# nkwangyh/CubemapSLAM

Measured on AMD Instinct MI355X. Metric: frames/sec (extract+match+localBA) on Lafida cam0, higher is better.
Workload: dtype u8 (extract/match), f64 (BA)

## Files before the change

cubemapslam_amd/csrc/cms_api_ba.hip:

```cpp
#include <algorithm>
#include <cfloat>
#include <chrono>
#include <condition_variable>
#include <deque>
#include <functional>
#include <atomic>
#include <cmath>
#include <mutex>
#include <numeric>
#include <string>
#include <thread>
#include <pthread.h>
#include <unordered_map>
#include "cms_ba_pool.h"

struct BaKnobs {
  bool deterministic, det_points, host_lm, single_host_lm, schur_chunks, schur_points, all_lists, want_all_lists;
  bool no_fused, solve1, trial_points, fixed_ranges, no_permute, create_timing, compose_timing, runs, runs_as_edges, separate_reduce, separate_reduce2, separate_first_pass, rm_valu;
  int solve_reduce_max, leftover_lookahead;
  bool global_sum;
  int lookahead, compose_segments, dup, run_min_chunks, rm_weight, se_waves_cap, em_cost_a, em_cost_b, te_chunks, run_min_pct; bool unified;
  char stream_priority;
  bool run_wg; int rw_waves_cu0, rw_waves_cu1;
};
static const BaKnobs& ba_knobs() {
  static const BaKnobs k = [] {
    BaKnobs q;
    auto on = [](const char* n) { return getenv(n) != nullptr; };
    auto num = [](const char* n, int dflt) { const char* v = getenv(n); return v ? atoi(v) : dflt; };
    q.deterministic = on("CMS_BA_DETERMINISTIC"); q.host_lm = on("CMS_BA_HOST_LM"); q.single_host_lm = on("CMS_BA_SINGLE_HOST_LM");
    q.schur_chunks = on("CMS_BA_SCHUR_CHUNKS"); q.schur_points = on("CMS_BA_SCHUR_POINTS"); q.all_lists = on("CMS_BA_ALL_LISTS");
    q.det_points = on("CMS_BA_DET_POINTS");
    q.want_all_lists = (q.deterministic && q.det_points) || q.host_lm || q.single_host_lm || q.schur_chunks || q.schur_points || q.all_lists;
    q.no_fused = on("CMS_BA_NO_FUSED_LIN"); q.solve1 = on("CMS_BA_SOLVE1"); q.trial_points = on("CMS_BA_TRIAL_POINTS");
    q.fixed_ranges = on("CMS_BA_FIXED_RANGES"); q.no_permute = on("CMS_BA_NO_PERMUTE");
    q.create_timing = on("CMS_BA_CREATE_TIMING"); q.compose_timing = on("CMS_BA_COMPOSE_TIMING");
    q.runs = !on("CMS_BA_NO_RUNS");
    q.runs_as_edges = on("CMS_BA_RUNS_AS_EDGES");
    q.rm_valu = on("CMS_BA_RM_VALU");
    q.separate_first_pass = on("CMS_BA_SEPARATE_FIRST_PASS");
    q.separate_reduce2 = on("CMS_BA_SEPARATE_REDUCE2");
    q.separate_reduce = on("CMS_BA_SEPARATE_REDUCE");
    { const char* v = getenv("CMS_BA_SOLVE_REDUCE_MAX"); q.solve_reduce_max = v ? atoi(v) : 24; }
    q.global_sum = !on("CMS_BA_NO_GLOBAL_SUM");
    q.leftover_lookahead = num("CMS_BA_LEFTOVER_LOOKAHEAD", 0);
    q.lookahead = num("CMS_BA_LOOKAHEAD", 24); q.compose_segments = num("CMS_BA_COMPOSE_SEGMENTS", 0); q.dup = num("CMS_BA_DUP", 0);
    q.run_min_chunks = std::max(1, num("CMS_BA_RUN_MIN_CHUNKS", q.rm_valu ? 2 : 1));
    q.run_min_pct = std::max(10, std::min(100, num("CMS_BA_RUN_MIN_PCT", 100)));
    q.rm_weight = std::max(10, std::min(400, num("CMS_BA_RM_WEIGHT", 58)));
    q.unified = !on("CMS_BA_SPLIT_WORKGROUPS");
    q.em_cost_a = num("CMS_BA_EM_COST_A", 40); q.em_cost_b = num("CMS_BA_EM_COST_B", 30);
    q.te_chunks = std::max(1, std::min(16, num("CMS_BA_TE_CHUNKS", 2)));
    q.se_waves_cap = num("CMS_BA_SE_WAVES", 0);
    q.run_wg = on("CMS_BA_RUN_WG");
    q.rw_waves_cu0 = std::max(1, std::min(32, num("CMS_BA_RW_WAVES0", 12))); q.rw_waves_cu1 = std::max(1, std::min(32, num("CMS_BA_RW_WAVES1", 8)));
    const char* pr = getenv("CMS_BA_STREAM_PRIORITY");
    q.stream_priority = pr ? pr[0] : 0;
    return q;
  }();
  return k;
}

struct BaExpand;
struct BaDevPlan;
struct BaCreateOpts {
  hipStream_t setup_stream = nullptr;
  bool inputs_pinned = false;
  bool force_host_plan = false;
  BaDevPlan* dev_plan = nullptr;
  BaExpand* defer_expand = nullptr;
};
struct BaCreated { bool expand_deferred = false; };
struct cms_ba {
  int device = 0;
  hipStream_t stream = nullptr; bool own_stream = true, pooled_stream = false;
  int K = 0, P = 0, E = 0, np = 0, nblk_e = 0, nblk_p = 0;
  std::vector<int> perm;
  std::vector<int> pinv;
  std::vector<int> se_chunk_pt0;
  BaDev d;
  uint8_t* d_fixed = nullptr; int* d_pose_slot = nullptr; int* d_e_pose = nullptr; int* d_e_point = nullptr;
  double* d_e_obs = nullptr; double* d_e_inv = nullptr; int8_t* d_e_face = nullptr; int* d_pt_off = nullptr;
  double* d_raw_obs = nullptr; double* d_raw_inv = nullptr; double* d_raw_pts = nullptr; int* d_perm = nullptr; int* d_pinv = nullptr;
  int* d_pose_off = nullptr; int* d_pose_edges = nullptr; uint8_t* d_level = nullptr; double* d_err = nullptr; double* d_ow = nullptr;
  double* d_poses[2] = {nullptr, nullptr}; double* d_pts[2] = {nullptr, nullptr};
  double* d_poses0 = nullptr; double* d_pts0 = nullptr;
  double* d_Hpp = nullptr; double* d_bp = nullptr; double* d_Hll = nullptr; double* d_bl = nullptr; double* d_Hpl = nullptr;
  double* d_Dinv = nullptr; double* d_Hs = nullptr; double* d_bs = nullptr; double* d_x = nullptr; double* d_Dg = nullptr;
// ... 16 lines not shown
  int cur = 0;
  double* h_pin = nullptr; size_t h_pin_bytes = 0;
  void* grp_items_dev = nullptr; void* grp_items_host = nullptr; double* grp_scal_dev = nullptr; double* grp_scal_host = nullptr;
  void* grp_lm_dev = nullptr; void* grp_lm_host = nullptr;
  int grp_cap = 0;
  int prof_kernel = 0; std::vector<hipEvent_t> prof_ev; double prof_ms = 0; long prof_launches = 0;
  bool fast_plan = false;
  int* d_raw_pose = nullptr; int* d_raw_point = nullptr; int8_t* d_raw_face = nullptr; int* d_prank = nullptr; int* d_cpo = nullptr; int* d_cedge = nullptr;
  uint8_t* d_pcopy = nullptr; uint8_t* d_lo_copy = nullptr; uint64_t* d_run_sig = nullptr; int* d_iperm = nullptr;
  bool dev_plan = false;
  int* d_plan_counts = nullptr; int* h_plan_counts = nullptr; size_t h_plan_counts_bytes = 0;
  long long* d_plan_clk = nullptr;
  bool se_only = false;
  bool deterministic = false;
  int det_ranges = 0;
  bool det_points = false;
  hipEvent_t ev_setup = nullptr;
  bool setup_wait_pending = false;
  hipStream_t grp_stream = nullptr;
  bool async_pending = false;
  bool gsum_clean = false;
  BaSe grp_se = {};
  std::vector<BaBlock> slabs; size_t slab_off = 0;
  size_t grp_pin_bytes[3] = {0, 0, 0};
};

#define BA_LDS_CEILING (160 * 1024 - 512)
static int ba_lds_attrs_once(int device) {
  static std::mutex mu;
  static bool done[64] = {false};
  std::lock_guard<std::mutex> lk(mu);
  if (device < 0 || device >= 64 || done[device]) return CMS_OK;
  const void* fns[] = {(const void*)k_ba_schur_points, (const void*)kb_ba_schur_points, (const void*)kb_ba_schur_edges, (const void*)kb_ba_lin_schur_edges,
                       (const void*)kb_ba_lin_schur_runs, (const void*)kb_ba_lin_schur_runs_det, (const void*)kb_ba_lin_schur_edges_det, (const void*)kb_ba_lin_schur_runs_valu, (const void*)kb_ba_lin_schur_run_wg0, (const void*)kb_ba_lin_schur_run_wg1, (const void*)kb_ba_trial_solve3r, (const void*)kb_ba_trial_solve3rp, (const void*)k_ba_trial_solve,
                       (const void*)kb_ba_trial_solve, (const void*)kb_ba_trial_solve3, (const void*)k_ba_solve_r192};
  for (const void* f : fns) {
    hipError_t e = hipFuncSetAttribute(f, hipFuncAttributeMaxDynamicSharedMemorySize, BA_LDS_CEILING);
    if (e != hipSuccess) return cms_fail(CMS_ERR_HIP, "hipFuncSetAttribute(MaxDynamicSharedMemorySize)", e);
  }
  done[device] = true;
  return CMS_OK;
}

struct BaPools {
  static size_t slab_cap() { const char* v = getenv("CMS_BA_POOL_MB"); return v ? (size_t)std::max(0, atoi(v)) << 20 : (size_t)16 << 30; }
  BaIdleList<hipStream_t> streams{256}, setup_streams{0};
  BaIdleList<hipEvent_t> events{1024};
  BaBlockCache dev{slab_cap(), 0};
  BaBlockCache pin{(size_t)2 << 30, 512}, stage{(size_t)2 << 30, 512};
};
static BaPools& ba_pools() { static BaPools* p = new BaPools; return *p; }
static hipStream_t ba_stream_take(int device) { return ba_pools().streams.take(device); }
static hipError_t ba_wait_stream(hipStream_t s) {
  static const bool relaxed = getenv("CMS_BA_RELAXED_WAIT") != nullptr;
  if (!relaxed) return hipStreamSynchronize(s);
  for (int i = 0; i < 64; ++i) {
    const hipError_t q = hipStreamQuery(s);
    if (q != hipErrorNotReady) return q == hipSuccess ? hipStreamSynchronize(s) : q;
  }
  for (;;) {
    std::this_thread::sleep_for(std::chrono::microseconds(40));
    const hipError_t q = hipStreamQuery(s);
    if (q != hipErrorNotReady) return q == hipSuccess ? hipStreamSynchronize(s) : q;
  }
}
static void ba_stream_give(int device, hipStream_t s) {
  const hipError_t q = hipStreamQuery(s);
  if ((q != hipSuccess && q != hipErrorNotReady) || !ba_pools().streams.give(device, s)) hipStreamDestroy(s);
// ... 1568 lines not shown
```

cubemapslam_amd/csrc/cms_api_ba_lm.hip:

```cpp

struct BaLm {
  int iterations = 0, robust = 0;
  double delta = 0;
  int it = 0, qmax = 0, nBad = 0, done = 0, next = 0;
  double lambda = -1, ni = 2, currentChi = 0, iniChi = 0, rho = 0;
  double chi_ini = 0, chi_fin = 0, lam_fin = 0;
};

static bool ba_stopped(const volatile uint8_t* stop) { return stop && *stop; }

static int ba_enqueue_iter_start(cms_ba* b, const BaLm& st) {
  hipStream_t s = b->stream;
  const int cur = b->cur;
  ba_errors(b, cur, st.robust, st.delta, 0);
  hipLaunchKernelGGL(k_ba_lin_points, dim3(b->nblk_p), dim3(128), 0, s, b->d, (const double*)b->d_poses[cur],
                     (const double*)b->d_pts[cur], st.robust, st.delta, b->d_Hll, b->d_bl, b->d_Hpl);
  hipLaunchKernelGGL(k_ba_lin_poses, dim3(b->K, BA_POSE_CHUNKS), dim3(256), 0, s, b->d, (const double*)b->d_poses[cur],
                     (const double*)b->d_pts[cur], st.robust, st.delta, b->d_pose_partial);
  if (b->np > 0)
    hipLaunchKernelGGL(k_ba_pose_finish, dim3(b->np), dim3(64), 0, s, b->np, (const double*)b->d_pose_partial, b->d_Hpp, b->d_bp);
  if (st.it == 0) {
    HIPCHK(hipMemsetAsync(b->d_scal + 3, 0, sizeof(double), s));
    hipLaunchKernelGGL(k_ba_maxdiag, dim3(64), dim3(256), 0, s, b->np, b->P, (const double*)b->d_Hpp, (const double*)b->d_Hll, b->d_scal + 3);
  }
// ... 338 lines not shown
  BaDyn dyn{};
  memset(&dyn, 0, sizeof(dyn));
  dyn.robust = st[0].robust; dyn.delta = st[0].delta; dyn.chi2_th = 5.991; dyn.set_level = 0; dyn.dev_lm = 1; dyn.fold_finish = 1;
  bool first_round = false;
  for (int w = 0; w < n; ++w) first_round = first_round || st[w].it == 0;
  const BaGroupMode gm = ba_group_mode(bas, n);
  const bool use_se = gm.use_se, use_te = gm.use_te;
  bool iter_phase = true;
  const bool use_s3 = gm.use_s3;
  int s3_threads = 64; size_t lds3 = 0;
  for (int w = 0; w < n; ++w) { s3_threads = std::max(s3_threads, ba_s3_threads(bas[w]->np)); lds3 = std::max(lds3, bas[w]->blk3_lds); }
  {
    static const int solve_kb = [] { const char* v = getenv("CMS_BA_SOLVE_LDS_KB"); return v ? atoi(v) : 0; }();
    if (solve_kb > 0) lds3 = std::max(lds3, std::min((size_t)solve_kb * 1024, (size_t)BA_LDS_CEILING));
  }
  int max_seR = 0, max_np2 = 0, max_Rt = 0; size_t se_lds = 0, te_lds = 0, rm_lds = 0;
  const int se_waves = gm.se_waves;
  bool any_runs = false, any_rw0 = false, any_rw1 = false;
  for (int w = 0; w < n; ++w) {
    const BaSe& gs = bas[w]->grp_se;
    if (gm.run_wg) { any_rw0 = any_rw0 || gs.n_rmA > 0; any_rw1 = any_rw1 || gs.n_rm > gs.n_rmA; }
    max_seR = std::max(max_seR, gs.R_rm + gs.R); max_np2 = std::max(max_np2, gs.npairs2); se_lds = std::max(se_lds, bas[w]->se_lds_fixed);
    any_runs = any_runs || gs.R_rm > 0;
    if (gs.R_rm > 0) rm_lds = std::max(rm_lds, bas[w]->rm_lds);
    max_Rt = std::max(max_Rt, gs.Rt); te_lds = std::max(te_lds, ((size_t)24 * bas[w]->K + 6 * (size_t)std::max(bas[w]->np, 1)) * sizeof(double));
  }
  se_lds += (size_t)se_waves * ((size_t)64 * 18 * sizeof(double) + 64 * sizeof(int));
  se_lds = std::max(se_lds, rm_lds);
  const int se_threads = 64 * se_waves;
  const size_t rw_lds = ba_rw_lds(std::max(max_K, 1));
  const int rw_units0 = std::max(8, std::min(BA_RW_CUTS, ba_device_cus(bas[0]->device) * ba_knobs().rw_waves_cu0 / std::max(n, 1)));
  const int rw_units1 = std::max(8, std::min(BA_RW_CUTS, ba_device_cus(bas[0]->device) * ba_knobs().rw_waves_cu1 / std::max(n, 1)));
  const bool fused = gm.fused;
  const bool solve_reduces = fused && (gm.gsum || (!ba_knobs().separate_reduce && max_seR <= ba_knobs().solve_reduce_max));
  dyn.fused_lin = fused ? 1 : 0;
  {
    static const bool no_presum = getenv("CMS_BA_NO_SOLVE_PRESUM") != nullptr;
    const size_t need = lds3 + (size_t)max_np2 * 42 * sizeof(double);
    if (use_s3 && solve_reduces && !gm.gsum && !no_presum && need <= BA_LDS_CEILING) { dyn.solve_presum = 1; lds3 = need; }
  }
  const bool first_pass = fused && use_te && first_round && !ba_knobs().separate_first_pass;
  dyn.fold_reduce = (use_te && !ba_knobs().separate_reduce2 && ba_knobs().dup == 0) ? 1 : 0;
  int k = 0;
  const int pk = g->prof_kernel;
  const int dup = ba_knobs().dup;
  auto bracket = [&](int id, int which) {
    if (pk != id) return;
    const size_t i = 2 * (size_t)k + which;
    while (g->prof_ev.size() <= i) { hipEvent_t e = nullptr; if (hipEventCreate(&e) != hipSuccess) return; g->prof_ev.push_back(e); }
    hipEventRecord(g->prof_ev[i], s);
  };
  auto enqueue_round = [&]() {
      if (first_round && first_pass) {
        bracket(1, 0);
        hipLaunchKernelGGL(kb_ba_first_pass, dim3(max_Rt, 1, n), dim3(BA_TE_THREADS), te_lds, s, ditems, dyn, (int)BA_PHASE_ITER);
        bracket(1, 1);
        iter_phase = false;
      } else if (first_round) {
        hipLaunchKernelGGL(kb_ba_errors, dim3(max_e, 1, n), dim3(256), 0, s, ditems, dyn, (int)BA_PHASE_ITER);
        hipLaunchKernelGGL(kb_ba_reduce, dim3(1, 1, n), dim3(256), 0, s, ditems, dyn, (int)BA_PHASE_ITER);
      }
      first_round = false;
      if (iter_phase) {
        const int npb = (max_P + 255) / 256;
        bracket(1, 0);
        hipLaunchKernelGGL(kb_ba_lin, dim3(npb + max_K * BA_POSE_CHUNKS, 1, n), dim3(256), 0, s, ditems, dyn, (int)BA_PHASE_ITER, npb);
// ... 15 lines not shown
          if (any_rw1) hipLaunchKernelGGL(kb_ba_lin_schur_run_wg1, dim3(rw_units1, 1, n), dim3(64), rw_lds, s, ditems, dyn, (int)BA_PHASE_TRIAL, rw_units1);
          if (any_rw0) hipLaunchKernelGGL(kb_ba_lin_schur_run_wg0, dim3(rw_units0, 1, n), dim3(64), rw_lds, s, ditems, dyn, (int)BA_PHASE_TRIAL, rw_units0);
          if (max_seR > 0) hipLaunchKernelGGL(kb_ba_lin_schur_edges, dim3(max_seR, 1, n), dim3(se_threads), se_lds, s, ditems, dyn, (int)BA_PHASE_TRIAL);
        } else if (fused && gm.det) {
          if (any_runs) hipLaunchKernelGGL(kb_ba_lin_schur_runs_det, dim3(max_seR, 1, n), dim3(se_threads), se_lds, s, ditems, dyn, (int)BA_PHASE_TRIAL);
          else hipLaunchKernelGGL(kb_ba_lin_schur_edges_det, dim3(max_seR, 1, n), dim3(se_threads), se_lds, s, ditems, dyn, (int)BA_PHASE_TRIAL);
        } else if (fused && any_runs) {
          hipLaunchKernelGGL(kb_ba_lin_schur_runs, dim3(max_seR, 1, n), dim3(se_threads), se_lds, s, ditems, dyn, (int)BA_PHASE_TRIAL);
          if (dup == 3) hipLaunchKernelGGL(kb_ba_lin_schur_runs, dim3(max_seR, 1, n), dim3(se_threads), se_lds, s, ditems, dyn, (int)BA_PHASE_TRIAL);
        } else if (fused) {
          hipLaunchKernelGGL(kb_ba_lin_schur_edges, dim3(max_seR, 1, n), dim3(se_threads), se_lds, s, ditems, dyn, (int)BA_PHASE_TRIAL);
          if (dup == 3) hipLaunchKernelGGL(kb_ba_lin_schur_edges, dim3(max_seR, 1, n), dim3(se_threads), se_lds, s, ditems, dyn, (int)BA_PHASE_TRIAL);
        } else {
          hipLaunchKernelGGL(kb_ba_schur_edges, dim3(max_seR, 1, n), dim3(se_threads), se_lds, s, ditems, dyn, (int)BA_PHASE_TRIAL);
          if (dup == 3) hipLaunchKernelGGL(kb_ba_schur_edges, dim3(max_seR, 1, n), dim3(se_threads), se_lds, s, ditems, dyn, (int)BA_PHASE_TRIAL);
        }
        bracket(3, 1);
        bracket(4, 0);
        if (!solve_reduces) hipLaunchKernelGGL(kb_ba_schur_edges_reduce, dim3(max_np2, 1, n), dim3(256), 0, s, ditems, dyn, (int)BA_PHASE_TRIAL);
        bracket(4, 1);
      } else if (all_sp) {
        bracket(3, 0);
        hipLaunchKernelGGL(kb_ba_schur_points, dim3(max_R, 1, n), dim3(max_spt), sp_lds, s, ditems, dyn, (int)BA_PHASE_TRIAL);
        if (dup == 3) hipLaunchKernelGGL(kb_ba_schur_points, dim3(max_R, 1, n), dim3(max_spt), sp_lds, s, ditems, dyn, (int)BA_PHASE_TRIAL);
        bracket(3, 1);
        bracket(4, 0);
        hipLaunchKernelGGL(kb_ba_schur_reduce, dim3(max_pairs, 1, n), dim3(256), 0, s, ditems, dyn, (int)BA_PHASE_TRIAL);
        if (dup == 4) hipLaunchKernelGGL(kb_ba_schur_reduce, dim3(max_pairs, 1, n), dim3(256), 0, s, ditems, dyn, (int)BA_PHASE_TRIAL);
        bracket(4, 1);
      } else if (max_chunks > 0) {
        hipLaunchKernelGGL(kb_ba_schur_chunks, dim3(max_chunks, 1, n), dim3(256), 0, s, ditems, dyn, (int)BA_PHASE_TRIAL);
      }
      bracket(5, 0);
      if (use_s3 && solve_reduces && dyn.solve_presum) {
        hipLaunchKernelGGL(kb_ba_trial_solve3rp, dim3(1, 1, n), dim3(s3_threads), lds3, s, ditems, dyn, (int)BA_PHASE_TRIAL);
      } else if (use_s3 && solve_reduces) {
        hipLaunchKernelGGL(kb_ba_trial_solve3r, dim3(1, 1, n), dim3(s3_threads), lds3, s, ditems, dyn, (int)BA_PHASE_TRIAL);
        if (dup == 5) hipLaunchKernelGGL(kb_ba_trial_solve3r, dim3(1, 1, n), dim3(s3_threads), lds3, s, ditems, dyn, (int)BA_PHASE_TRIAL);
      } else if (use_s3) {
        hipLaunchKernelGGL(kb_ba_trial_solve3, dim3(1, 1, n), dim3(s3_threads), lds3, s, ditems, dyn, (int)BA_PHASE_TRIAL);
        if (dup == 5) hipLaunchKernelGGL(kb_ba_trial_solve3, dim3(1, 1, n), dim3(s3_threads), lds3, s, ditems, dyn, (int)BA_PHASE_TRIAL);
      } else {
        hipLaunchKernelGGL(kb_ba_trial_solve, dim3(1, 1, n), dim3(384), lds, s, ditems, dyn, (int)BA_PHASE_TRIAL);
        if (dup == 5) hipLaunchKernelGGL(kb_ba_trial_solve, dim3(1, 1, n), dim3(384), lds, s, ditems, dyn, (int)BA_PHASE_TRIAL);
      }
      bracket(5, 1);
      bracket(6, 0);
      if (use_te) {
        hipLaunchKernelGGL(kb_ba_trial_edges, dim3(max_Rt, 1, n), dim3(BA_TE_THREADS), te_lds, s, ditems, dyn, (int)BA_PHASE_TRIAL);
        if (dup == 6) hipLaunchKernelGGL(kb_ba_trial_edges, dim3(max_Rt, 1, n), dim3(BA_TE_THREADS), te_lds, s, ditems, dyn, (int)BA_PHASE_TRIAL);
      } else {
        hipLaunchKernelGGL(kb_ba_trial_points, dim3(max_p, 1, n), dim3(128), 0, s, ditems, dyn, (int)BA_PHASE_TRIAL);
        if (dup == 6) hipLaunchKernelGGL(kb_ba_trial_points, dim3(max_p, 1, n), dim3(128), 0, s, ditems, dyn, (int)BA_PHASE_TRIAL);
      }
      bracket(6, 1);
      bracket(7, 0);
      if (!dyn.fold_reduce) hipLaunchKernelGGL(kb_ba_reduce2, dim3(1, 1, n), dim3(256), 0, s, ditems, dyn, (int)BA_PHASE_TRIAL);
      bracket(7, 1);
      ++k;
  };
  const volatile BaLmDev* vh = reinterpret_cast<const volatile BaLmDev*>(hlm);
  hipError_t werr = hipSuccess;
  for (long spins = 0;;) {
    bool any = false;
    for (int w = 0; w < n; ++w) any = any || vh[w].next != 2;
    if (!any || (k > 0 && ba_stopped(stop))) break;
    if (k - vh[0].rounds < (stop ? 1 : 2)) { enqueue_round(); spins = 0; continue; }
    if (spins < 256) std::this_thread::yield();
    else std::this_thread::sleep_for(std::chrono::microseconds(20));
    if ((++spins & 0xFFF) == 0 && hipStreamQuery(s) != hipErrorNotReady) {
      werr = hipStreamSynchronize(s);
      if (werr != hipSuccess || k - vh[0].rounds >= 2) { if (werr == hipSuccess) werr = hipErrorUnknown; break; }
    }
  }
// ... 168 lines not shown
```

cubemapslam_amd/csrc/cms_ba_fused.hip:

```cpp
#include <hip/hip_runtime.h>
#include <stdint.h>

__device__ __forceinline__ void ba_factor_diag(double* a, int J, double* Ld, double* ybuf, double* idg, int* bad) {
  double idl[6];
#pragma unroll
  for (int c = 0; c < 6; ++c) {
    const double dc = a[7 * c];
    if (!(isfinite(dc)) || dc == 0.0) *bad = 1;
    double x = __builtin_amdgcn_rcp(dc);
    x = __builtin_fma(__builtin_fma(-dc, x, 1.0), x, x);
    x = __builtin_fma(__builtin_fma(-dc, x, 1.0), x, x);
    idl[c] = x;
    double lc[6];
#pragma unroll
    for (int r = c + 1; r < 6; ++r) lc[r] = a[6 * r + c] * x;
#pragma unroll
    for (int r = c + 1; r < 6; ++r) {
#pragma unroll
      for (int q = c + 1; q <= r; ++q) a[6 * r + q] = __builtin_fma(-lc[r], a[6 * q + c], a[6 * r + q]);
    }
#pragma unroll
    for (int r = c + 1; r < 6; ++r) a[6 * r + c] = lc[r];
  }
  double z[6];
#pragma unroll
  for (int r = 0; r < 6; ++r) z[r] = ybuf[6 * J + r];
#pragma unroll
  for (int r = 0; r < 6; ++r) {
#pragma unroll
    for (int c = 0; c < r; ++c) z[r] = __builtin_fma(-a[6 * r + c], z[c], z[r]);
  }
#pragma unroll
  for (int r = 1; r < 6; ++r)
#pragma unroll
    for (int c = 0; c < r; ++c) Ld[6 * r + c] = a[6 * r + c];
#pragma unroll
  for (int r = 0; r < 6; ++r) { ybuf[6 * J + r] = z[r]; idg[6 * J + r] = idl[r]; }
}

__device__ __forceinline__ void ba_trial_pose_update(BaDevG d, const double* ybuf, const double* __restrict__ bp, double lambda, const double* __restrict__ poses,
                                                     double* __restrict__ poses_new, double* __restrict__ scal, bool isbad) {
  const int tid = threadIdx.x;
  double sc = 0;
  for (int k = tid; k < d.K; k += blockDim.x) {
    const double* T = poses + 7 * k;
    double* Tn = poses_new + 7 * k;
    const int s = d.pose_slot[k];
    if (s < 0) { for (int i = 0; i < 7; ++i) Tn[i] = T[i]; continue; }
    const double* u = ybuf + 6 * s;
    for (int i = 0; i < 6; ++i) sc += u[i] * (lambda * u[i] + bp[6 * s + i]);
    const double om[3] = {u[0], u[1], u[2]}, up[3] = {u[3], u[4], u[5]};
    const double theta = sqrt(om[0] * om[0] + om[1] * om[1] + om[2] * om[2]);
    const double Om[9] = {0, -om[2], om[1], om[2], 0, -om[0], -om[1], om[0], 0};
    double Om2[9];
    for (int i = 0; i < 3; ++i)
      for (int j = 0; j < 3; ++j) Om2[3 * i + j] = Om[3 * i] * Om[j] + Om[3 * i + 1] * Om[3 + j] + Om[3 * i + 2] * Om[6 + j];
    double R[9], V[9];
    if (theta < 0.00001) {
      for (int i = 0; i < 9; ++i) { R[i] = ((i & 3) == 0 ? 1.0 : 0.0) + Om[i] + Om2[i]; V[i] = R[i]; }
    } else {
      double sn, cs;
      sincos(theta, &sn, &cs);
      const double sa = sn / theta, sb = (1 - cs) / (theta * theta), scc = (theta - sn) / (theta * theta * theta);
      for (int i = 0; i < 9; ++i) {
        const double Id = ((i & 3) == 0 ? 1.0 : 0.0);
        R[i] = Id + sa * Om[i] + sb * Om2[i];
        V[i] = Id + sb * Om[i] + scc * Om2[i];
      }
    }
    double Eq[4], Et[3], RE[9];
// ... 177 lines not shown
      }
      for (int o = tid; o < 6 * J; o += 64) {
        const int Kq = o / 6, c = o - 6 * Kq;
        const int mq = nb - Kq - 1, iq = J - Kq - 1;
        const double* Lq = Lp + 36 * (size_t)(Kq * nb - Kq * (Kq + 1) / 2);
        double v = ybuf[o];
#pragma unroll
        for (int r = 0; r < 6; ++r) { const int q = 6 * r + c; v -= Lq[((q >> 1) * mq + iq) * 2 + (q & 1)] * xj[r]; }
        ybuf[o] = v;
      }
      __builtin_amdgcn_wave_barrier();
    }
  }
  __syncthreads();
  if (isbad) for (int i = tid; i < n; i += blockDim.x) ybuf[i] = 0.0;
  __syncthreads();
  BA_CLK(3);
  for (int i = tid; i < n; i += blockDim.x) xp_out[i] = ybuf[i];
  ba_trial_pose_update(d, ybuf, bp, lambda, poses, poses_new, scal, isbad);
  BA_CLK(4);
#undef BA_CLK
}

#define BA_S3_STRIDE 38
#define BA_S3_BPW 21
#define BA_S3_NY 3
static inline int ba_s3_threads(int np) { return (np * (np + 1) / 2 + BA_S3_BPW - 1) / BA_S3_BPW * 64; }
#ifdef BA_S3_CLK
__device__ long long ba_s3_clk[16];
#define BA_S3_STAMP(i) do { if (s3_on) { const long long now_ = (long long)__builtin_readcyclecounter(); s3_acc[i] += now_ - s3_last; s3_last = now_; } } while (0)
#else
#define BA_S3_STAMP(i) do { } while (0)
#endif
__device__ __forceinline__ void ba_trial_solve3_body(BaDevG d, const double* __restrict__ Hpp, const double* __restrict__ bp, double lambda,
                 const int* __restrict__ pair_of_block, const int* __restrict__ pair_chunk_off,
                 const double* __restrict__ chunk_sum, const double* __restrict__ poses, double* __restrict__ poses_new,
                 double* __restrict__ xp_out, double* __restrict__ scal, bool lumped = false, double* partial = nullptr,
                 double* bp_partial = nullptr, int n_slices = 0, int NP2 = 0, bool consume = false, bool presum = false) {
  extern __shared__ __align__(16) double sm[];
  const int nb = d.np, n = 6 * nb, nblk = nb * (nb + 1) / 2;
  double* Lp = sm;
  double* Ldg = Lp + (size_t)BA_S3_STRIDE * (nb * (nb - 1) / 2);
  double* Wbuf = Ldg + 36 * (size_t)nb;
  double* dstage = Wbuf + 2 * (size_t)BA_S3_STRIDE * nb;
  double* ybuf = dstage + 36;
  double* idg = ybuf + n;
  double* bps = idg + n;
  double* ssum = bps + n;
  const bool presummed = partial && presum && !consume && n_slices > 1;
  if (presummed) {
    const int tot = NP2 * 42;
    for (int i = threadIdx.x; i < tot; i += blockDim.x) {
      double v = 0.0;
#pragma unroll 8
      for (int r = 0; r < n_slices; ++r) v += partial[(size_t)r * tot + i];
      ssum[i] = v;
    }
    __syncthreads();
  }
#ifdef BA_S3_CLK
  const bool s3_on = threadIdx.x == 0 && blockIdx.z == 0;
  long long s3_acc[10] = {0, 0, 0, 0, 0, 0, 0, 0, 0, 0};
  long long s3_last = (long long)__builtin_readcyclecounter();
#endif
  if (partial) {
    for (int i = threadIdx.x; i < n; i += blockDim.x) {
// ... 44 lines not shown
        if (I == K && consume) {
#pragma unroll
          for (int q = 0; q < 6; ++q) {
            a[q] -= cs[6 * min(q, r0) + max(q, r0)];
            a[6 + q] -= cs[6 * min(q, r0 + 1) + max(q, r0 + 1)];
          }
        } else {
#pragma unroll
          for (int q = 0; q < 6; ++q) { const double2 v = *reinterpret_cast<const double2*>(cs + 6 * q + r0); a[q] -= v.x; a[6 + q] -= v.y; }
        }
        if (I == K) { const double2 v = *reinterpret_cast<const double2*>(cs + 36 + r0); yb[0] += v.x; yb[1] += v.y; }
        if (consume) {
#pragma unroll
          for (int q = 0; q < 6; ++q) *reinterpret_cast<double2*>(cs + 6 * q + r0) = make_double2(0.0, 0.0);
          if (I == K) *reinterpret_cast<double2*>(cs + 36 + r0) = make_double2(0.0, 0.0);
        }
      }
    } else if (pr >= 0) {
      for (int c = pair_chunk_off[pr]; c < pair_chunk_off[pr + 1]; ++c) {
        const double* cs = chunk_sum + (size_t)c * 42;
#pragma unroll
        for (int q = 0; q < 6; ++q) { a[q] -= cs[6 * q + r0]; a[6 + q] -= cs[6 * q + r0 + 1]; }
        if (I == K) { yb[0] += cs[36 + r0]; yb[1] += cs[36 + r0 + 1]; }
      }
    }
    if (I == K) {
      ybuf[6 * I + r0] = (lumped ? 0.0 : bp[6 * I + r0]) - yb[0];
      ybuf[6 * I + r0 + 1] = (lumped ? 0.0 : bp[6 * I + r0 + 1]) - yb[1];
    }
  }
#define BA_S3_WAVE_SYNC() do { __builtin_amdgcn_fence(__ATOMIC_RELEASE, "wavefront"); __builtin_amdgcn_wave_barrier(); \
                               __builtin_amdgcn_fence(__ATOMIC_ACQUIRE, "wavefront"); } while (0)
  if (wave == 0) {
    if (have && I == 0 && K == 0) {
#pragma unroll
      for (int q = 0; q < 12; ++q) dstage[6 * r0 + q] = a[q];
    }
    BA_S3_WAVE_SYNC();
    if (tid == 0) {
      double f[36];
#pragma unroll
      for (int q = 0; q < 36; ++q) f[q] = dstage[q];
      ba_factor_diag(f, 0, Ldg, ybuf, idg, &bad);
    }
  }
  __syncthreads();
  BA_S3_STAMP(0);
  for (int J = 0; J < nb && !bad; ++J) {
    double* Wp = Wbuf + (size_t)(J & 1) * BA_S3_STRIDE * nb;
    double* Lpan = Lp + (size_t)BA_S3_STRIDE * (J * nb - J * (J + 1) / 2);
    if (have && K == J && I > J) {
      const double* Ld = Ldg + 36 * (size_t)J;
      double ld[15], idj[6], zj[6];
#pragma unroll
      for (int c = 1; c < 6; ++c)
#pragma unroll
        for (int q = 0; q < c; ++q) ld[c * (c - 1) / 2 + q] = Ld[6 * c + q];
#pragma unroll
      for (int c = 0; c < 6; ++c) { idj[c] = idg[6 * J + c]; zj[c] = ybuf[6 * J + c]; }
      double yi[2] = {ybuf[6 * I + r0], ybuf[6 * I + r0 + 1]};
      double w[12], lo[12];
#pragma unroll
      for (int r = 0; r < 2; ++r)
#pragma unroll
        for (int c = 0; c < 6; ++c) {
          double v = a[6 * r + c];
#pragma unroll
          for (int q = 0; q < c; ++q) v = __builtin_fma(-w[6 * r + q], ld[c * (c - 1) / 2 + q], v);
          w[6 * r + c] = v;
        }
#pragma unroll
      for (int r = 0; r < 2; ++r)
#pragma unroll
        for (int c = 0; c < 6; ++c) {
          const double l = w[6 * r + c] * idj[c];
          lo[6 * r + c] = l;
          yi[r] = __builtin_fma(-l, zj[c], yi[r]);
        }
      const int i = I - J - 1;
      double2* W2 = reinterpret_cast<double2*>(Wp + (size_t)i * BA_S3_STRIDE + 6 * r0);
      double2* L2 = reinterpret_cast<double2*>(Lpan + (size_t)i * BA_S3_STRIDE + 6 * r0);
#pragma unroll
      for (int q = 0; q < 6; ++q) { W2[q] = make_double2(w[2 * q], w[2 * q + 1]); L2[q] = make_double2(lo[2 * q], lo[2 * q + 1]); }
      ybuf[6 * I + r0] = yi[0]; ybuf[6 * I + r0 + 1] = yi[1];
    }
    __syncthreads();
    BA_S3_STAMP(2);
    const bool next_diag = have && I == J + 1 && K == J + 1;
    const int blkd = (J + 1) * nb - (J + 1) * J / 2, wd = blkd / BA_S3_BPW;
    const bool crit = J + 1 < nb && wave == wd;
    if (crit) __builtin_amdgcn_s_setprio(3);
    if (have && K > J) {
      const int iw = I - J - 1, ik = K - J - 1;
      double wv[12], lk[36];
      const double2* W2 = reinterpret_cast<const double2*>(Wp + (size_t)iw * BA_S3_STRIDE + 6 * r0);
      const double2* L2 = reinterpret_cast<const double2*>(Lpan + (size_t)ik * BA_S3_STRIDE);
#pragma unroll
      for (int q = 0; q < 6; ++q) { const double2 x = W2[q]; wv[2 * q] = x.x; wv[2 * q + 1] = x.y; }
#pragma unroll
      for (int q = 0; q < 18; ++q) { const double2 y = L2[q]; lk[2 * q] = y.x; lk[2 * q + 1] = y.y; }
#pragma unroll
      for (int r = 0; r < 2; ++r)
#pragma unroll
        for (int q = 0; q < 6; ++q) {
          double v = a[6 * r + q];
#pragma unroll
          for (int c = 0; c < 6; ++c) v = __builtin_fma(-wv[6 * r + c], lk[6 * q + c], v);
          a[6 * r + q] = v;
        }
      if (next_diag) {
#pragma unroll
        for (int q = 0; q < 12; ++q) dstage[6 * r0 + q] = a[q];
      }
    }
    if (crit) {
      BA_S3_WAVE_SYNC();
      if (lane == 3 * (blkd - BA_S3_BPW * wd)) {
        double f[36];
#pragma unroll
        for (int q = 0; q < 36; ++q) f[q] = dstage[q];
        ba_factor_diag(f, J + 1, Ldg + 36 * (size_t)(J + 1), ybuf, idg, &bad);
      }
      __builtin_amdgcn_s_setprio(0);
    }
    __syncthreads();
    BA_S3_STAMP(3);
  }
  const bool isbad = bad != 0;
  if (!isbad && wave == 0) {
    const int ln = min(lane, 59);
    double y[BA_S3_NY];
    const double* Lo[BA_S3_NY];
#pragma unroll
    for (int g = 0; g < BA_S3_NY; ++g) {
      const int o = 60 * g + ln;
      y[g] = o < n ? ybuf[o] * idg[o] : 0.0;
      const int Kq = o / 6, c = o - 6 * Kq;
      Lo[g] = Lp + (ptrdiff_t)BA_S3_STRIDE * (Kq * nb - Kq * (Kq + 1) / 2 - Kq - 1) + c;
    }
    const double* Lsafe = Lp - BA_S3_STRIDE;
    double nld[15];
    auto fetch = [&](int J) {
      const double* Ld = Ldg + 36 * (size_t)J;
#pragma unroll
      for (int q = 1; q < 6; ++q)
#pragma unroll
        for (int r = 0; r < q; ++r) nld[q * (q - 1) / 2 + r] = Ld[6 * q + r];
    };
// ... 140 lines not shown
```

cubemapslam_amd/csrc/cms_ba_wrappers.hip:

```cpp
#include <hip/hip_runtime.h>
#include <stdint.h>

#define BA_MAX_GROUP 64
struct BaLmDev {
  double lambda, ni, currentChi, iniChi, rho, chi_ini, chi_fin, lam_fin;
  int it, iterations, qmax, nBad, done, next, cur, rounds;
  int n_out[2], pad[2];
};
struct BaItem {
  BaDev d;
  double* poses[2]; double* pts[2];
  double* Hll; double* bl; double* Hpl; double* Hpp; double* bp; double* pose_partial; double* Dinv; double* db;
  double* chunk_sum; double* x; double* partial; double* scal;
  double* hscal;
  const int2* chunk_range; const int2* tup; const int* pair_of_block; const int* pair_chunk_off;
  uint8_t* flags;
  int nblk_e, nblk_p, nchunks, block_free;
  BaSp sp;
  BaSe se;
  BaLmDev* lm; BaLmDev* hlm;
};
template <class T> struct BaGP {
  BA_AS1 T* p;
  __device__ __forceinline__ BaGP() {}
// ... 241 lines not shown
  ba_schur_edges_body<true, true>(blockIdx.x, it.d, it.se, it.Hll, it.bl, ba_lambda, it.poses[cur], it.pts[cur], dyn.robust, dyn.delta);
}
extern "C" __global__ void __launch_bounds__(BA_SE_THREADS) kb_ba_lin_schur_runs_valu(const BaItem* __restrict__ items, BaDyn dyn, int phase) {
  BA_ITEM(phase, it.se.R_rm + it.se.R)
  if ((int)blockIdx.x < it.se.R_rm) ba_schur_runs_body(blockIdx.x, it.d, it.se, it.Hll, it.bl, ba_lambda, it.poses[cur], it.pts[cur], dyn.robust, dyn.delta);
  else ba_schur_edges_body<true>((int)blockIdx.x - it.se.R_rm, it.d, it.se, it.Hll, it.bl, ba_lambda, it.poses[cur], it.pts[cur], dyn.robust, dyn.delta);
}
extern "C" __global__ void __launch_bounds__(256) kb_ba_schur_edges_reduce(const BaItem* __restrict__ items, BaDyn dyn, int phase) {
  BA_ITEM(phase, it.se.nchunks > 0 ? it.se.npairs2 : 0)
  BaSpG v;
  v.R = it.se.R_rm + it.se.R; v.npairs = it.se.npairs2; v.partial = it.se.partial;
  ba_schur_reduce_body(blockIdx.x, v, it.chunk_sum);
  if (dyn.fused_lin && (int)blockIdx.x < it.d.np) {
    __shared__ double bps[6 * BA_SE_RANGES];
    const int R = min(it.se.R_rm + it.se.R, BA_SE_RANGES);
    for (int t = threadIdx.x; t < 6 * R; t += blockDim.x) bps[t] = it.se.bp_partial[((size_t)(t / 6) * it.d.np + blockIdx.x) * 6 + (t % 6)];
    __syncthreads();
    if (threadIdx.x < 6) {
      double sum = 0.0;
      for (int r = 0; r < R; ++r) sum += bps[6 * r + threadIdx.x];
      it.bp[6 * blockIdx.x + threadIdx.x] = sum;
    }
  }
}
extern "C" __global__ void __launch_bounds__(256) kb_ba_schur_reduce(const BaItem* __restrict__ items, BaDyn dyn, int phase) {
  BA_ITEM(phase, it.sp.R > 0 ? it.sp.npairs : 0)
  ba_schur_reduce_body(blockIdx.x, it.sp, it.chunk_sum);
}
extern "C" __global__ void __launch_bounds__(384) kb_ba_trial_solve(const BaItem* __restrict__ items, BaDyn dyn, int phase) {
  BA_ITEM(phase, 1)
  ba_trial_solve_body(0, 1, it.d, it.Hpp, it.bp, ba_lambda, it.pair_of_block, it.pair_chunk_off, it.chunk_sum, it.poses[cur], it.poses[nxt],
                      it.x, it.scal);
}
extern "C" __global__ void __launch_bounds__(1024) kb_ba_trial_solve3(const BaItem* __restrict__ items, BaDyn dyn, int phase) {
  BA_ITEM(phase, 1)
  ba_trial_solve3_body(it.d, it.Hpp, it.bp, ba_lambda, it.pair_of_block, it.pair_chunk_off, it.chunk_sum, it.poses[cur], it.poses[nxt], it.x, it.scal,
                       dyn.fused_lin != 0);
}
extern "C" __global__ void __launch_bounds__(1024) kb_ba_trial_solve3r(const BaItem* __restrict__ items, BaDyn dyn, int phase) {
  BA_ITEM(phase, 1)
  ba_trial_solve3_body(it.d, it.Hpp, it.bp, ba_lambda, it.pair_of_block, it.pair_chunk_off, it.chunk_sum, it.poses[cur], it.poses[nxt], it.x, it.scal,
                       true, (double*)it.se.partial, (double*)it.se.bp_partial, it.se.gsum ? 1 : it.se.R_rm + it.se.R, it.se.npairs2, it.se.gsum != 0, false);
}
extern "C" __global__ void __launch_bounds__(1024) kb_ba_trial_solve3rp(const BaItem* __restrict__ items, BaDyn dyn, int phase) {
  BA_ITEM(phase, 1)
  ba_trial_solve3_body(it.d, it.Hpp, it.bp, ba_lambda, it.pair_of_block, it.pair_chunk_off, it.chunk_sum, it.poses[cur], it.poses[nxt], it.x, it.scal,
                       true, (double*)it.se.partial, (double*)it.se.bp_partial, it.se.R_rm + it.se.R, it.se.npairs2, false, true);
}
extern "C" __global__ void __launch_bounds__(128) kb_ba_trial_points(const BaItem* __restrict__ items, BaDyn dyn, int phase) {
  BA_ITEM(phase, it.nblk_p)
  ba_trial_points_body(blockIdx.x, it.nblk_p, it.d, it.bl, it.Hpl, it.Dinv, it.x, ba_lambda, it.pts[cur], it.pts[nxt], it.poses[nxt], dyn.robust,
                       dyn.delta, it.partial, it.block_free ? it.Hll : nullptr, it.block_free ? it.poses[cur] : nullptr);
}
__device__ __forceinline__ void ba_round_count(const BaItem* __restrict__ items) {
  BaLmDev* L0 = items[0].lm;
  const int r = L0->rounds + 1;
  L0->rounds = r;
  *reinterpret_cast<volatile int*>(&items[0].hlm->rounds) = r;
}
__device__ __forceinline__ void ba_trial_publish(const BaItemG& it, const BaDyn& dyn) {
  if (dyn.dev_lm && threadIdx.x == 0) {
    const int ok2 = (int)__double_as_longlong(it.scal[4]);
    ba_lm_after_trial(it.lm, it.hlm, it.scal[1], it.scal[2], ok2, dyn.fused_lin != 0);
  }
}
#define BA_TICKET_SLOT 7
extern "C" __global__ void __launch_bounds__(BA_TE_THREADS) kb_ba_trial_edges(const BaItem* __restrict__ items, BaDyn dyn, int phase) {
  if (dyn.fold_reduce && dyn.dev_lm && blockIdx.z == 0 && blockIdx.x == 0 && threadIdx.x == 0 && (items[0].lm->next != 1 || items[0].se.Rt < 1)) ba_round_count(items);
  BA_ITEM(phase, it.se.Rt)
  ba_trial_edges_body(blockIdx.x, it.se.Rt, it.d, it.se, it.bl, it.Hll, it.x, ba_lambda, it.pts[cur], it.pts[nxt], it.poses[cur], it.poses[nxt], dyn.robust,
                      dyn.delta, it.partial, dyn.fold_reduce != 0);
  if (!dyn.fold_reduce) return;
  __shared__ int last_sh;
  __shared__ double sh2[16];
  const int n = it.se.Rt;
  int* ticket = reinterpret_cast<int*>((double*)it.scal + BA_TICKET_SLOT);
  if (threadIdx.x == 0) last_sh = atomicAdd(ticket, 1) == n - 1;
  __syncthreads();
  if (!last_sh) return;
  double* partial = it.partial;
// ... 89 lines not shown
```

Baseline: 24770.

## Parallelize 6x6 diagonal Cholesky across lanes in solve3 and add 640-thread variants

Replaces the single-thread 6x6 diagonal-block factorization in the trial solve kernel with a cooperative version spread over three lanes (two rows each), using readlane broadcasts and a refined reciprocal. This removes the LDS staging and wave sync on the critical path of the blocked Cholesky. It also adds kernel variants with launch bounds of 640 to allow more registers when fewer threads are used, selected through a lookup table. The old path remains behind an environment knob; the refined-rcp reciprocal may differ slightly numerically from a division.

```diff
diff --git a/cubemapslam_amd/csrc/cms_api_ba.hip b/cubemapslam_amd/csrc/cms_api_ba.hip
--- a/cubemapslam_amd/csrc/cms_api_ba.hip
+++ b/cubemapslam_amd/csrc/cms_api_ba.hip
@@ -22,6 +22,7 @@
   int lookahead, compose_segments, dup, run_min_chunks, rm_weight, se_waves_cap, em_cost_a, em_cost_b, te_chunks, run_min_pct; bool unified;
   char stream_priority;
   bool run_wg; int rw_waves_cu0, rw_waves_cu1;
+  bool solve3_generic;
 };
 static const BaKnobs& ba_knobs() {
   static const BaKnobs k = [] {
@@ -54,6 +55,7 @@
     q.se_waves_cap = num("CMS_BA_SE_WAVES", 0);
     q.run_wg = on("CMS_BA_RUN_WG");
     q.rw_waves_cu0 = std::max(1, std::min(32, num("CMS_BA_RW_WAVES0", 12))); q.rw_waves_cu1 = std::max(1, std::min(32, num("CMS_BA_RW_WAVES1", 8)));
+    q.solve3_generic = num("CMS_BA_SOLVE3_GENERIC", 0) != 0;
     const char* pr = getenv("CMS_BA_STREAM_PRIORITY");
     q.stream_priority = pr ? pr[0] : 0;
     return q;
@@ -136,8 +138,12 @@
   std::lock_guard<std::mutex> lk(mu);
   if (device < 0 || device >= 64 || done[device]) return CMS_OK;
   const void* fns[] = {(const void*)k_ba_schur_points, (const void*)kb_ba_schur_points, (const void*)kb_ba_schur_edges, (const void*)kb_ba_lin_schur_edges,
-                       (const void*)kb_ba_lin_schur_runs, (const void*)kb_ba_lin_schur_runs_det, (const void*)kb_ba_lin_schur_edges_det, (const void*)kb_ba_lin_schur_runs_valu, (const void*)kb_ba_lin_schur_run_wg0, (const void*)kb_ba_lin_schur_run_wg1, (const void*)kb_ba_trial_solve3r, (const void*)kb_ba_trial_solve3rp, (const void*)k_ba_trial_solve,
-                       (const void*)kb_ba_trial_solve, (const void*)kb_ba_trial_solve3, (const void*)k_ba_solve_r192};
+                       (const void*)kb_ba_lin_schur_runs, (const void*)kb_ba_lin_schur_runs_det, (const void*)kb_ba_lin_schur_edges_det, (const void*)kb_ba_lin_schur_runs_valu, (const void*)kb_ba_lin_schur_run_wg0, (const void*)kb_ba_lin_schur_run_wg1, (const void*)k_ba_trial_solve,
+                       (const void*)kb_ba_trial_solve, (const void*)k_ba_solve_r192,
+#define BA_X(NAME) (const void*)NAME, (const void*)NAME##_640, (const void*)NAME##_generic,
+                       BA_SOLVE3_ALL(BA_X)
+#undef BA_X
+  };
   for (const void* f : fns) {
     hipError_t e = hipFuncSetAttribute(f, hipFuncAttributeMaxDynamicSharedMemorySize, BA_LDS_CEILING);
     if (e != hipSuccess) return cms_fail(CMS_ERR_HIP, "hipFuncSetAttribute(MaxDynamicSharedMemorySize)", e);
diff --git a/cubemapslam_amd/csrc/cms_api_ba_lm.hip b/cubemapslam_amd/csrc/cms_api_ba_lm.hip
--- a/cubemapslam_amd/csrc/cms_api_ba_lm.hip
+++ b/cubemapslam_amd/csrc/cms_api_ba_lm.hip
@@ -394,6 +394,7 @@
   const int rw_units0 = std::max(8, std::min(BA_RW_CUTS, ba_device_cus(bas[0]->device) * ba_knobs().rw_waves_cu0 / std::max(n, 1)));
   const int rw_units1 = std::max(8, std::min(BA_RW_CUTS, ba_device_cus(bas[0]->device) * ba_knobs().rw_waves_cu1 / std::max(n, 1)));
   const bool fused = gm.fused;
+  const bool s3_generic = ba_knobs().solve3_generic;
   const bool solve_reduces = fused && (gm.gsum || (!ba_knobs().separate_reduce && max_seR <= ba_knobs().solve_reduce_max));
   dyn.fused_lin = fused ? 1 : 0;
   {
@@ -475,14 +476,11 @@
         hipLaunchKernelGGL(kb_ba_schur_chunks, dim3(max_chunks, 1, n), dim3(256), 0, s, ditems, dyn, (int)BA_PHASE_TRIAL);
       }
       bracket(5, 0);
-      if (use_s3 && solve_reduces && dyn.solve_presum) {
-        hipLaunchKernelGGL(kb_ba_trial_solve3rp, dim3(1, 1, n), dim3(s3_threads), lds3, s, ditems, dyn, (int)BA_PHASE_TRIAL);
-      } else if (use_s3 && solve_reduces) {
-        hipLaunchKernelGGL(kb_ba_trial_solve3r, dim3(1, 1, n), dim3(s3_threads), lds3, s, ditems, dyn, (int)BA_PHASE_TRIAL);
-        if (dup == 5) hipLaunchKernelGGL(kb_ba_trial_solve3r, dim3(1, 1, n), dim3(s3_threads), lds3, s, ditems, dyn, (int)BA_PHASE_TRIAL);
-      } else if (use_s3) {
-        hipLaunchKernelGGL(kb_ba_trial_solve3, dim3(1, 1, n), dim3(s3_threads), lds3, s, ditems, dyn, (int)BA_PHASE_TRIAL);
-        if (dup == 5) hipLaunchKernelGGL(kb_ba_trial_solve3, dim3(1, 1, n), dim3(s3_threads), lds3, s, ditems, dyn, (int)BA_PHASE_TRIAL);
+      if (use_s3) {
+        const bool presum = solve_reduces && dyn.solve_presum;
+        const BaSolve3Kernel solve3 = ba_solve3_kernel(presum ? 2 : solve_reduces ? 1 : 0, s3_threads, s3_generic);
+        hipLaunchKernelGGL(solve3, dim3(1, 1, n), dim3(s3_threads), lds3, s, ditems, dyn, (int)BA_PHASE_TRIAL);
+        if (dup == 5 && !presum) hipLaunchKernelGGL(solve3, dim3(1, 1, n), dim3(s3_threads), lds3, s, ditems, dyn, (int)BA_PHASE_TRIAL);
       } else {
         hipLaunchKernelGGL(kb_ba_trial_solve, dim3(1, 1, n), dim3(384), lds, s, ditems, dyn, (int)BA_PHASE_TRIAL);
         if (dup == 5) hipLaunchKernelGGL(kb_ba_trial_solve, dim3(1, 1, n), dim3(384), lds, s, ditems, dyn, (int)BA_PHASE_TRIAL);
diff --git a/cubemapslam_amd/csrc/cms_ba_fused.hip b/cubemapslam_amd/csrc/cms_ba_fused.hip
--- a/cubemapslam_amd/csrc/cms_ba_fused.hip
+++ b/cubemapslam_amd/csrc/cms_ba_fused.hip
@@ -36,6 +36,49 @@
     for (int c = 0; c < r; ++c) Ld[6 * r + c] = a[6 * r + c];
 #pragma unroll
   for (int r = 0; r < 6; ++r) { ybuf[6 * J + r] = z[r]; idg[6 * J + r] = idl[r]; }
+}
+
+__device__ __forceinline__ double ba_readlane_f64(double v, int l) {
+  return __hiloint2double(__builtin_amdgcn_readlane(__double2hiint(v), l), __builtin_amdgcn_readlane(__double2loint(v), l));
+}
+__device__ __forceinline__ void ba_factor_diag3(double* a, int base, int rp, int J, double* Ld, double* ybuf, double* idg, int* bad) {
+  const int r0 = 2 * rp;
+  double z[2], ix[2] = {0.0, 0.0};
+  {
+    const double2 v = *reinterpret_cast<const double2*>(ybuf + 6 * J + r0);
+    z[0] = v.x; z[1] = v.y;
+  }
+  bool isbad = false;
+#pragma unroll
+  for (int c = 0; c < 6; ++c) {
+    const int lc_ = base + (c >> 1);
+    const double dc = ba_readlane_f64(a[6 * (c & 1) + c], lc_);
+    double col[6];
+#pragma unroll
+    for (int q = c + 1; q < 6; ++q) col[q] = ba_readlane_f64(a[6 * (q & 1) + c], base + (q >> 1));
+    const double zc = ba_readlane_f64(z[c & 1], lc_);
+    if (!(isfinite(dc)) || dc == 0.0) isbad = true;
+    double x = __builtin_amdgcn_rcp(dc);
+    x = __builtin_fma(__builtin_fma(-dc, x, 1.0), x, x);
+    x = __builtin_fma(__builtin_fma(-dc, x, 1.0), x, x);
+    if (rp == (c >> 1)) ix[c & 1] = x;
+#pragma unroll
+    for (int t = 0; t < 2; ++t) {
+      if (4 + t <= c) continue;
+      const bool below = r0 + t > c;
+      const double l = a[6 * t + c] * x;
+#pragma unroll
+      for (int q = c + 1; q <= 4 + t; ++q) a[6 * t + q] = __builtin_fma(-l, col[q], a[6 * t + q]);
+      a[6 * t + c] = below ? l : a[6 * t + c];
+      z[t] = below ? __builtin_fma(-l, zc, z[t]) : z[t];
+    }
+  }
+  double2* L2 = reinterpret_cast<double2*>(Ld + 6 * r0);
+#pragma unroll
+  for (int q = 0; q < 6; ++q) L2[q] = make_double2(a[2 * q], a[2 * q + 1]);
+  *reinterpret_cast<double2*>(ybuf + 6 * J + r0) = make_double2(z[0], z[1]);
+  *reinterpret_cast<double2*>(idg + 6 * J + r0) = make_double2(ix[0], ix[1]);
+  if (isbad && rp == 0) *bad = 1;
 }
 
 __device__ __forceinline__ void ba_trial_pose_update(BaDevG d, const double* ybuf, const double* __restrict__ bp, double lambda, const double* __restrict__ poses,
@@ -279,6 +322,7 @@
 #else
 #define BA_S3_STAMP(i) do { } while (0)
 #endif
+template <bool DIAG3>
 __device__ __forceinline__ void ba_trial_solve3_body(BaDevG d, const double* __restrict__ Hpp, const double* __restrict__ bp, double lambda,
                  const int* __restrict__ pair_of_block, const int* __restrict__ pair_chunk_off,
                  const double* __restrict__ chunk_sum, const double* __restrict__ poses, double* __restrict__ poses_new,
@@ -389,16 +433,20 @@
 #define BA_S3_WAVE_SYNC() do { __builtin_amdgcn_fence(__ATOMIC_RELEASE, "wavefront"); __builtin_amdgcn_wave_barrier(); \
                                __builtin_amdgcn_fence(__ATOMIC_ACQUIRE, "wavefront"); } while (0)
   if (wave == 0) {
-    if (have && I == 0 && K == 0) {
-#pragma unroll
-      for (int q = 0; q < 12; ++q) dstage[6 * r0 + q] = a[q];
-    }
-    BA_S3_WAVE_SYNC();
-    if (tid == 0) {
-      double f[36];
-#pragma unroll
-      for (int q = 0; q < 36; ++q) f[q] = dstage[q];
-      ba_factor_diag(f, 0, Ldg, ybuf, idg, &bad);
+    if (DIAG3) {
+      if (have && blk == 0) ba_factor_diag3(a, 0, rp, 0, Ldg, ybuf, idg, &bad);
+    } else {
+      if (have && I == 0 && K == 0) {
+#pragma unroll
+        for (int q = 0; q < 12; ++q) dstage[6 * r0 + q] = a[q];
+      }
+      BA_S3_WAVE_SYNC();
+      if (tid == 0) {
+        double f[36];
+#pragma unroll
+        for (int q = 0; q < 36; ++q) f[q] = dstage[q];
+        ba_factor_diag(f, 0, Ldg, ybuf, idg, &bad);
+      }
     }
   }
   __syncthreads();
@@ -465,12 +513,16 @@
           for (int c = 0; c < 6; ++c) v = __builtin_fma(-wv[6 * r + c], lk[6 * q + c], v);
           a[6 * r + q] = v;
         }
-      if (next_diag) {
+      if (!DIAG3 && next_diag) {
 #pragma unroll
         for (int q = 0; q < 12; ++q) dstage[6 * r0 + q] = a[q];
       }
     }
-    if (crit) {
+    if (crit && DIAG3) {
+      const int bd = blkd - BA_S3_BPW * wd;
+      if (next_diag) ba_factor_diag3(a, 3 * bd, rp, J + 1, Ldg + 36 * (size_t)(J + 1), ybuf, idg, &bad);
+      __builtin_amdgcn_s_setprio(0);
+    } else if (crit) {
       BA_S3_WAVE_SYNC();
       if (lane == 3 * (blkd - BA_S3_BPW * wd)) {
         double f[36];
diff --git a/cubemapslam_amd/csrc/cms_ba_wrappers.hip b/cubemapslam_amd/csrc/cms_ba_wrappers.hip
--- a/cubemapslam_amd/csrc/cms_ba_wrappers.hip
+++ b/cubemapslam_amd/csrc/cms_ba_wrappers.hip
@@ -297,20 +297,30 @@
   ba_trial_solve_body(0, 1, it.d, it.Hpp, it.bp, ba_lambda, it.pair_of_block, it.pair_chunk_off, it.chunk_sum, it.poses[cur], it.poses[nxt],
                       it.x, it.scal);
 }
-extern "C" __global__ void __launch_bounds__(1024) kb_ba_trial_solve3(const BaItem* __restrict__ items, BaDyn dyn, int phase) {
-  BA_ITEM(phase, 1)
-  ba_trial_solve3_body(it.d, it.Hpp, it.bp, ba_lambda, it.pair_of_block, it.pair_chunk_off, it.chunk_sum, it.poses[cur], it.poses[nxt], it.x, it.scal,
-                       dyn.fused_lin != 0);
-}
-extern "C" __global__ void __launch_bounds__(1024) kb_ba_trial_solve3r(const BaItem* __restrict__ items, BaDyn dyn, int phase) {
-  BA_ITEM(phase, 1)
-  ba_trial_solve3_body(it.d, it.Hpp, it.bp, ba_lambda, it.pair_of_block, it.pair_chunk_off, it.chunk_sum, it.poses[cur], it.poses[nxt], it.x, it.scal,
-                       true, (double*)it.se.partial, (double*)it.se.bp_partial, it.se.gsum ? 1 : it.se.R_rm + it.se.R, it.se.npairs2, it.se.gsum != 0, false);
-}
-extern "C" __global__ void __launch_bounds__(1024) kb_ba_trial_solve3rp(const BaItem* __restrict__ items, BaDyn dyn, int phase) {
-  BA_ITEM(phase, 1)
-  ba_trial_solve3_body(it.d, it.Hpp, it.bp, ba_lambda, it.pair_of_block, it.pair_chunk_off, it.chunk_sum, it.poses[cur], it.poses[nxt], it.x, it.scal,
-                       true, (double*)it.se.partial, (double*)it.se.bp_partial, it.se.R_rm + it.se.R, it.se.npairs2, false, true);
+#define BA_SOLVE3_KERNELS(NAME, ...) \
+  extern "C" __global__ void __launch_bounds__(1024) NAME(const BaItem* __restrict__ items, BaDyn dyn, int phase) { \
+    BA_ITEM(phase, 1) \
+    ba_trial_solve3_body<true>(it.d, it.Hpp, it.bp, ba_lambda, it.pair_of_block, it.pair_chunk_off, it.chunk_sum, it.poses[cur], it.poses[nxt], it.x, it.scal, __VA_ARGS__); \
+  } \
+  extern "C" __global__ void __launch_bounds__(640) NAME##_640(const BaItem* __restrict__ items, BaDyn dyn, int phase) { \
+    BA_ITEM(phase, 1) \
+    ba_trial_solve3_body<true>(it.d, it.Hpp, it.bp, ba_lambda, it.pair_of_block, it.pair_chunk_off, it.chunk_sum, it.poses[cur], it.poses[nxt], it.x, it.scal, __VA_ARGS__); \
+  } \
+  extern "C" __global__ void __launch_bounds__(1024) NAME##_generic(const BaItem* __restrict__ items, BaDyn dyn, int phase) { \
+    BA_ITEM(phase, 1) \
+    ba_trial_solve3_body<false>(it.d, it.Hpp, it.bp, ba_lambda, it.pair_of_block, it.pair_chunk_off, it.chunk_sum, it.poses[cur], it.poses[nxt], it.x, it.scal, __VA_ARGS__); \
+  }
+BA_SOLVE3_KERNELS(kb_ba_trial_solve3, dyn.fused_lin != 0)
+BA_SOLVE3_KERNELS(kb_ba_trial_solve3r, true, (double*)it.se.partial, (double*)it.se.bp_partial, it.se.gsum ? 1 : it.se.R_rm + it.se.R, it.se.npairs2, it.se.gsum != 0, false)
+BA_SOLVE3_KERNELS(kb_ba_trial_solve3rp, true, (double*)it.se.partial, (double*)it.se.bp_partial, it.se.R_rm + it.se.R, it.se.npairs2, false, true)
+#undef BA_SOLVE3_KERNELS
+typedef void (*BaSolve3Kernel)(const BaItem*, BaDyn, int);
+#define BA_SOLVE3_ALL(X) X(kb_ba_trial_solve3) X(kb_ba_trial_solve3r) X(kb_ba_trial_solve3rp)
+static inline BaSolve3Kernel ba_solve3_kernel(int flavour, int threads, bool generic) {
+#define BA_X(NAME) {NAME, NAME##_640, NAME##_generic},
+  static const BaSolve3Kernel tab[3][3] = {BA_SOLVE3_ALL(BA_X)};
+#undef BA_X
+  return tab[flavour][generic ? 2 : threads <= 640 ? 1 : 0];
 }
 extern "C" __global__ void __launch_bounds__(128) kb_ba_trial_points(const BaItem* __restrict__ items, BaDyn dyn, int phase) {
   BA_ITEM(phase, it.nblk_p)
```

After: 24190. -2.3%, worse.
